# argsim/argsim

Measured on AMD Instinct MI355X. Metric: sentences/sec per ELBO step, higher is better.
Workload: dtype f32; 1 GPU; BASELINE configs[1]: 1xMI355X fp32, latent_dim 128, vocab 8k, seq_len 64, batch 256 per GPU; FULL synthetic Zipf batches, dim_emb 512, 3 layers, step 20000; global_batch=256, seq_len=64, parallelism=dp1, gru=persistent

## Files before the change

### argsim_amd/csrc/ctx.h

```cpp
#pragma once
#include "../../include/argsim_vae.h"
#include "kernels.h"

#include <fcntl.h>
#include <sys/file.h>
#include <unistd.h>

#include <algorithm>
#include <cmath>
#include <cstdio>
#include <cstring>
#include <string>
#include <vector>

#pragma GCC visibility push(hidden)
namespace avae { namespace host {

struct ParamEntry {
    std::string name;
    int64_t offset;
    int ndim;
    int64_t shape[4];
    int g16;
    int bucket;
// ... 7 lines not shown
struct avae_ctx {
    avae_config cfg{};
    int device = 0;
    hipStream_t stream = nullptr;
    std::string err;
    std::vector<avae::host::ParamEntry> params;
    int64_t numel = 0;
    std::vector<std::pair<int64_t, int64_t>> buckets;
    float *P = nullptr, *G = nullptr, *M = nullptr, *Vv = nullptr;
    int64_t step = 0;
    avae_grad_hook hook = nullptr; void* hook_user = nullptr;
    std::vector<int> hook_pending;
    int persistent = 1;
    bool first_step_checked = false;
    int gru_ablate = 0, gru_force_slow = 0, gru_stagger = 0, gru_item = 2;
    int skinny = 1;
    int score_plan[4] = {0, 0, 0, 0};
    const int* expect_ptr[3] = {nullptr, nullptr, nullptr}; int expect_val[3] = {0, 0, 0};
    int compact = 2;
    int skip_pad = 1;
    int shared_device = 0; int lock_fd = -1;
    int dyn_split = 1;
    int dyn_thin = 1;
    int enc_top1 = 1;
    int table_l1 = 1;
    int bf16_act = 1;
    int bf16_sv = 1;
    int bf16_tn = 1;
    int logits16 = 1;
    int bf16_nt8 = 1;
    int bf16_direct = 0;
    int gru_spec = 2;
    int bwd_rs = 2;
    int knn_chunk = 0;
    int gru_bf16 = 1;
    int64_t oE = 0, oKout = 0, oBout = 0, oWmu = 0, oBmu = 0, oWlv = 0, oBlv = 0, oWex = 0, oBex = 0;
    std::vector<avae::host::GruP> enc;
    std::vector<avae::host::GruP> dec;
    float* losses = nullptr;
    float* acc = nullptr;
    int* errw = nullptr;
    unsigned* counters = nullptr;
    float* scratch = nullptr;
    int64_t scratch_n = 0;
    char* ws = nullptr; size_t ws_cap = 0;
    int B = 0, Ss = 0, St = 0;
    int timing = 0, timing_on = 0;
    unsigned short *bfA = nullptr, *bfB = nullptr; size_t bfA_cap = 0, bfB_cap = 0;
    float* slab = nullptr; size_t slab_floats = 0;
    unsigned short* bfP = nullptr; size_t bfP_cap = 0;
    struct Stamp { hipEvent_t a, b; int cls; double flops; const int* dyn; int dyn_max; };
    std::vector<Stamp> stamps; size_t stamps_used = 0;
    int32_t* hint_dev = nullptr; volatile int32_t* hint_host = nullptr;
    const int32_t *cnt_src = nullptr, *cnt_tgt = nullptr;
};

#pragma GCC visibility push(hidden)
namespace avae { namespace host {

#define AV_CHECK(expr)                                                                              \
    do { hipError_t e_ = (expr); if (e_ != hipSuccess) {                                            \
        char b_[512]; snprintf(b_, sizeof b_, "%s:%d: %s -> %s", __FILE__, __LINE__, #expr, hipGetErrorString(e_)); \
        h->err = b_; return 1; } } while (0)
#define AV_TRY(expr) do { int r_ = (expr); if (r_) return r_; } while (0)

inline int fail(avae_ctx* h, const std::string& m) { h->err = m; return 1; }

#define AV_GRU(expr)                                                                                                \
    do { hipError_t e_ = (expr);                                                                                    \
         if (e_ == hipErrorCooperativeLaunchTooLarge)                                                               \
             return fail(h, "persistent GRU kernel: its workgroups cannot all be resident on this device at once (occupancy query x CU count < grid); " \
                            "run with avae_set_option(\"persistent\", 0)");                                         \
         if (e_ != hipSuccess) { char b_[512]; snprintf(b_, sizeof b_, "%s:%d: %s -> %s", __FILE__, __LINE__, #expr, hipGetErrorString(e_)); \
             h->err = b_; return 1; } } while (0)

struct DeviceTurn {
    avae_ctx* h; bool held = false;
    explicit DeviceTurn(avae_ctx* h_) : h(h_) {
        if (!h->shared_device || !h->persistent) return;
        if (h->lock_fd < 0) {
            char path[64]; snprintf(path, sizeof path, "/tmp/argsim_vae_dev%d.lock", h->device);
            h->lock_fd = open(path, O_CREAT | O_RDWR, 0666);
        }
        if (h->lock_fd >= 0 && flock(h->lock_fd, LOCK_EX) == 0) held = true;
    }
    ~DeviceTurn() { if (held) { (void)hipStreamSynchronize(h->stream); (void)flock(h->lock_fd, LOCK_UN); } }
};

struct Timed {
    avae_ctx* h; avae_ctx::Stamp* s = nullptr;
    Timed(avae_ctx* h_, int cls, double flops, const int* dyn = nullptr, int dyn_max = 0) : h(h_) {
        if (!h->timing) return;
        if (h->stamps_used == h->stamps.size()) {
            avae_ctx::Stamp n{};
            if (hipEventCreate(&n.a) != hipSuccess || hipEventCreate(&n.b) != hipSuccess) return;
            h->stamps.push_back(n);
        }
        s = &h->stamps[h->stamps_used++];
        s->cls = cls; s->flops = flops; s->dyn = dyn; s->dyn_max = dyn_max;
        (void)hipEventRecord(s->a, h->stream);
    }
    ~Timed() { if (s) (void)hipEventRecord(s->b, h->stream); }
};

struct Ws {
    int32_t *src_tm, *lens_src, *lens_tgt, *lead, *gold, *rank, *cidx, *ntok, *pred;
    float *emb_src, *emb_tgt, *ew, *dew;
    std::vector<float*> e_gi, e_hs, e_sv[2], e_hp[2];
    std::vector<float*> d_gi, d_hd, d_sv, d_hp;
    float *hpick, *mu, *lv, *z, *eps, *kld, *h0;
    float *xlast, *gib, *svb, *dgib, *dghb, *dxl;
    float *hc, *ho, *logits;
    float *loss_samp, *errt_samp;
    float *dho, *dhc, *dhd[2], *dgi_d, *dgh_d, *dh0, *carry, *dh0sum, *dz, *dmu, *dlv, *dhpick;
    float *dhs[2], *dgi_e, *dgh_e, *demb_src, *demb_tgt;
    std::vector<unsigned short*> e_hs16, d_hd16, e_hp16[2], d_hp16;
    std::vector<char> act_e, act_d, acth_e, acth_d;
    std::vector<unsigned short*> x16_e, x16_d;
    const unsigned short* x16_kept_e(int i) const { return x16_valid ? x16_e[i] : nullptr; }
    const unsigned short* x16_kept_d(int i) const { return x16_valid ? x16_d[i] : nullptr; }
    bool x16_valid = false;
    unsigned short *dgi16_d, *dgh16_d, *dgi16_e, *dgh16_e;
// ... 108 lines not shown
```

### argsim_amd/csrc/gemm_f32.hip

```cpp
#include "kernels.h"
#include <cstdlib>
#include <type_traits>

namespace avae {

typedef float f32x16 __attribute__((ext_vector_type(16)));

constexpr int BK = 32;
constexpr int LDK = BK + 4;

template <bool XC, int ROWS>
__device__ __forceinline__ void load_tile(float4 (&r)[ROWS / 32], const float* __restrict__ P, int ld,
                                          int x0, int X, int k0, int K1, int tid)
{
#pragma unroll
    for (int rep = 0; rep < ROWS / 32; ++rep) {
        int f = tid + 256 * rep;
        float4 v = make_float4(0.f, 0.f, 0.f, 0.f);
        if (XC) {
            int k = k0 + f / (ROWS / 4), x = x0 + ((f % (ROWS / 4)) << 2);
            if (k < K1 && x < X) v = *reinterpret_cast<const float4*>(P + (size_t)k * ld + x);
        } else {
            int x = x0 + (f >> 3), k = k0 + ((f & 7) << 2);
            if (x < X && k < K1) v = *reinterpret_cast<const float4*>(P + (size_t)x * ld + k);
// ... 77 lines not shown
        return;
    }
#pragma unroll
    for (int j = 0; j < TN; ++j) {
        int col = n0 + 32 * (wn * TN + j) + l31;
        if (col >= g.N) continue;
        float bv = add_bias ? g.bias[col] : 0.f;
#pragma unroll
        for (int i = 0; i < TM; ++i) {
#pragma unroll
            for (int r = 0; r < 16; ++r) {
                int row = m0 + 32 * (wm * TM + i) + (r & 3) + 8 * (r >> 2) + 4 * h;
                if (row >= M) continue;
                float v = g.alpha * acc[i][j][r] + bv;
                float* c = g.C + (size_t)row * g.ldc + col;
                if (atomic) atomicAdd(c, v);
                else if (g.accumulate) *c += v;
                else *c = v;
            }
        }
    }
}

template <bool A_MC, bool B_NC, int WM, int WN, int TM, int TN, bool FAST = false, bool DB = false>
__global__ __launch_bounds__(256, DB ? 2 : 3) void gemm_f32_kernel(GemmArgs g)
{
    constexpr int BM = 32 * WM * TM, BN = 32 * WN * TN;
    constexpr int kStage = (BM + BN) * LDK;
    __shared__ __attribute__((aligned(16))) float smem[kStage * (DB ? 2 : 1)];
    float* As = smem;
    float* Bs = smem + BM * LDK;

    const int tid = threadIdx.x, lane = tid & 63, wave = tid >> 6;
    const int h = lane >> 5, l31 = lane & 31;
    const int wm = wave / WN, wn = wave % WN;

    if (blockIdx.y) { g.A = g.A2; g.B = g.B2; g.C = g.C2; g.bias = g.bias2; }
    int M = g.M, K = g.K;
    if (g.dyn_kind == 1) M = min(M, *g.dyn);
    if (g.dyn_kind == 2) K = min(K, *g.dyn);

    const int tiles_n = (g.N + BN - 1) / BN;
    const int nblk = ((M + BM - 1) / BM) * tiles_n;
    int bid = blockIdx.x;
    {
        int q = nblk >> 3, r = nblk & 7, xcd = bid & 7, slot = bid >> 3;
        if (slot >= q + (xcd < r ? 1 : 0)) return;
        bid = (xcd < r ? xcd * (q + 1) : r * (q + 1) + (xcd - r) * q) + slot;
    }
    const int tm = bid / tiles_n, tn = bid - tm * tiles_n;
    const int m0 = tm * BM, n0 = tn * BN;
    if (m0 >= M) return;

    int kb = 0, ke = K;
    if (g.split_k > 1) {
        int ktiles = (K + BK - 1) / BK;
        int per = (ktiles + g.split_k - 1) / g.split_k;
        kb = blockIdx.z * per * BK;
        ke = min(K, kb + per * BK);
        if (kb >= ke) return;
// ... 88 lines not shown
}

template <bool A_MC, bool B_NC, bool FAST>
__global__ __launch_bounds__(256, 3) void gemm_f32_persist_kernel(GemmArgs g)
{
    static_assert(FAST, "buffer-load staging only (register budget of three workgroups per CU)");
    constexpr int TM = 2, TN = 2, WN = 2, BM = 128, BN = 128;
    __shared__ __attribute__((aligned(16))) float smem[(BM + BN) * LDK];
    float* As = smem;
    float* Bs = smem + BM * LDK;
    const int tid = threadIdx.x, lane = tid & 63, wave = tid >> 6;
    const int h = lane >> 5, l31 = lane & 31;
    const int wm = wave / WN, wn = wave % WN;

    int M = g.M;
    const int K = g.K;
    if (g.dyn_kind == 1) M = min(M, *g.dyn);
    const int tiles_n = (g.N + BN - 1) / BN;
    const int nblk = ((M + BM - 1) / BM) * tiles_n;
    const int xcd = blockIdx.x & 7, per_xcd = gridDim.x >> 3;
    const int q = nblk >> 3, r = nblk & 7;
    const int run0 = xcd < r ? xcd * (q + 1) : r * (q + 1) + (xcd - r) * q, run_n = q + (xcd < r ? 1 : 0);
    int local = blockIdx.x >> 3;
    if (local >= run_n) return;

    float4 ra[BM / 32], rb[BN / 32];
    FastTile<A_MC, BM> fa; FastTile<B_NC, BN> fb;
    auto first_tile = [&](int bid) __attribute__((always_inline)) {
        const int tm = bid / tiles_n, tn = bid - tm * tiles_n;
        if (FAST) {
            fa.init(g.A, g.lda, tm * BM, M, 0, K, tid); fb.init(g.B, g.ldb, tn * BN, g.N, 0, K, tid);
            fa.load(ra, 0); fb.load(rb, 0);
        } else {
            load_tile<A_MC, BM>(ra, g.A, g.lda, tm * BM, M, 0, K, tid);
            load_tile<B_NC, BN>(rb, g.B, g.ldb, tn * BN, g.N, 0, K, tid);
        }
    };
    first_tile(run0 + local);
    for (; local < run_n; local += per_xcd) {
        const int bid = run0 + local;
        const int tm = bid / tiles_n, tn = bid - tm * tiles_n;
        const int m0 = tm * BM, n0 = tn * BN;
        const bool more = local + per_xcd < run_n;
        f32x16 acc[TM][TN];
#pragma unroll
        for (int i = 0; i < TM; ++i)
#pragma unroll
            for (int j = 0; j < TN; ++j)
#pragma unroll
                for (int e = 0; e < 16; ++e) acc[i][j][e] = 0.f;
        for (int k0 = 0; k0 < K; k0 += BK) {
            store_tile<A_MC, BM>(As, ra, tid);
            store_tile<B_NC, BN>(Bs, rb, tid);
            if (k0 + BK < K) {
                if (FAST) { const int it = k0 / BK + 1; fa.load(ra, it); fb.load(rb, it); }
                else {
                    load_tile<A_MC, BM>(ra, g.A, g.lda, m0, M, k0 + BK, K, tid);
                    load_tile<B_NC, BN>(rb, g.B, g.ldb, n0, g.N, k0 + BK, K, tid);
                }
            } else if (more) {
                first_tile(bid + per_xcd);
// ... 16 lines not shown
#pragma unroll
                for (int t = 0; t < TN; ++t) {
                    if (B_NC) {
#pragma unroll
                        for (int e = 0; e < 4; ++e) b[t][e] = Bs[(8 * qq + 4 * h + e) * BN + 32 * (wn * TN + t) + l31];
                    } else {
                        float4 v = *reinterpret_cast<const float4*>(Bs + (32 * (wn * TN + t) + l31) * LDK + 8 * qq + 4 * h);
                        b[t][0] = v.x; b[t][1] = v.y; b[t][2] = v.z; b[t][3] = v.w;
                    }
                }
#pragma unroll
                for (int e = 0; e < 4; ++e)
#pragma unroll
                    for (int i = 0; i < TM; ++i)
#pragma unroll
                        for (int j = 0; j < TN; ++j)
                            acc[i][j] = __builtin_amdgcn_mfma_f32_32x32x2f32(a[i][e], b[j][e], acc[i][j], 0, 0, 0);
            }
            __builtin_amdgcn_s_setprio(0);
            __syncthreads();
        }
        epilogue<TM, TN, WN>(g, acc, M, m0, n0, BM, BN, wm, wn, h, l31, false, g.bias != nullptr);
    }
}

template <bool B_NC>
__global__ __launch_bounds__(512) void gemm_f32_skinny_kernel(GemmArgs g)
{
    __shared__ float red[7][16][64];
    if (blockIdx.y) { g.A = g.A2; g.B = g.B2; g.C = g.C2; g.bias = g.bias2; }
    const int tid = threadIdx.x, lane = tid & 63, wave = tid >> 6, l31 = lane & 31, h = lane >> 5;
    const int tiles_n = (g.N + 31) / 32, tm = blockIdx.x / tiles_n, tn = blockIdx.x - tm * tiles_n;
    const int m0 = tm * 32, n0 = tn * 32;
    const int kchunk = ((g.K + 63) / 64) * 8;
    const int k0 = wave * kchunk, k1 = min(g.K, k0 + kchunk);
    const float* __restrict__ ap = g.A + (size_t)min(m0 + l31, g.M - 1) * g.lda;
    const int bcol = min(n0 + l31, g.N - 1);
    const float* __restrict__ bp = B_NC ? g.B + bcol : g.B + (size_t)bcol * g.ldb;
    f32x16 acc;
#pragma unroll
    for (int r = 0; r < 16; ++r) acc[r] = 0.f;
    for (int kk = k0; kk < k1; kk += 32) {
        float4 a[4], b[4];
#pragma unroll
        for (int u = 0; u < 4; ++u) {
            const int k = kk + 8 * u + 4 * h;
// ... 40 lines not shown
    return !a_mc && g.split_k <= 1 && g.dyn_kind == 0 && (g.K & 3) == 0 && (g.lda & 3) == 0 && g.K >= 64;
}
static void launch_skinny(hipStream_t st, bool b_nc, const GemmArgs& g)
{
    dim3 grid(((g.M + 31) / 32) * ((g.N + 31) / 32), g.A2 ? 2 : 1);
    if (b_nc) hipLaunchKernelGGL(gemm_f32_skinny_kernel<true>, grid, dim3(512), 0, st, g);
    else      hipLaunchKernelGGL(gemm_f32_skinny_kernel<false>, grid, dim3(512), 0, st, g);
}

template <class F>
static void with_layouts(bool a_mc, bool b_nc, F&& f)
{
    if (!a_mc && !b_nc)      f(std::false_type{}, std::false_type{});
    else if (!a_mc && b_nc)  f(std::false_type{}, std::true_type{});
    else if (a_mc && b_nc)   f(std::true_type{}, std::true_type{});
    else                     f(std::true_type{}, std::false_type{});
}

template <int WM, int WN, int TM, int TN>
static void launch_variant(hipStream_t st, bool a_mc, bool b_nc, const GemmArgs& g)
{
    constexpr int BM = 32 * WM * TM, BN = 32 * WN * TN;
    int tiles = ((g.M + BM - 1) / BM) * ((g.N + BN - 1) / BN);
    dim3 grid(tiles, g.A2 ? 2 : 1, g.split_k > 1 ? g.split_k : 1);
    static const bool allow_fast = !getenv("AVAE_F32_NOFAST");
    const int k_per_wg = g.split_k > 1 ? (g.K + g.split_k - 1) / g.split_k : g.K;
    const bool fast = allow_fast && (a_mc ? (g.M % BM == 0) : (g.K % BK == 0 && g.dyn_kind != 2)) &&
                      (b_nc ? (g.N % BN == 0) : (g.K % BK == 0 && g.dyn_kind != 2)) && (a_mc || b_nc || k_per_wg >= 1536);
    static const char* ps_env = getenv("AVAE_F32_PERSIST");
    if constexpr (WM == 2 && WN == 2) {
        const bool aligned = (a_mc ? (g.M % BM == 0) : (g.K % BK == 0)) && (b_nc ? (g.N % BN == 0) : (g.K % BK == 0));
        const bool persist = (ps_env ? atoi(ps_env) != 0 : true) && allow_fast && aligned && !g.A2 && g.split_k <= 1 && g.dyn_kind != 2 && tiles > 1024;
        if (persist) {
            dim3 pg(768);
            with_layouts(a_mc, b_nc, [&](auto A, auto B) { hipLaunchKernelGGL((gemm_f32_persist_kernel<decltype(A)::value, decltype(B)::value, true>), pg, dim3(256), 0, st, g); });
            return;
        }
    }
    static const char* db_env = getenv("AVAE_F32_DB");
    if constexpr (WM == 2 && WN == 2) {
        const int eff_tiles = (g.dyn_kind == 1 && g.dyn_expect > 0) ? std::min(tiles, ((g.dyn_expect + BM - 1) / BM) * ((g.N + BN - 1) / BN)) : (g.dyn_kind == 1 ? 0 : tiles);
        const bool use_db = db_env ? atoi(db_env) != 0 && !g.A2 : (!g.A2 && g.split_k <= 1 && eff_tiles > 768 && tiles <= 1024);
        if (use_db) {
            if (fast) {
                with_layouts(a_mc, b_nc, [&](auto A, auto B) { hipLaunchKernelGGL((gemm_f32_kernel<decltype(A)::value, decltype(B)::value, WM, WN, TM, TN, true, true>), grid, dim3(256), 0, st, g); });
            } else {
                with_layouts(a_mc, b_nc, [&](auto A, auto B) { hipLaunchKernelGGL((gemm_f32_kernel<decltype(A)::value, decltype(B)::value, WM, WN, TM, TN, false, true>), grid, dim3(256), 0, st, g); });
            }
            return;
        }
    }
    if (fast) {
        with_layouts(a_mc, b_nc, [&](auto A, auto B) { hipLaunchKernelGGL((gemm_f32_kernel<decltype(A)::value, decltype(B)::value, WM, WN, TM, TN, true>), grid, dim3(256), 0, st, g); });
        return;
    }
    with_layouts(a_mc, b_nc, [&](auto A, auto B) { hipLaunchKernelGGL((gemm_f32_kernel<decltype(A)::value, decltype(B)::value, WM, WN, TM, TN>), grid, dim3(256), 0, st, g); });
}

hipError_t gemm_f32(hipStream_t st, bool a_mc, bool b_nc, const GemmArgs& g)
{
    if (g.M <= 0 || g.N <= 0) return hipSuccess;
    if ((g.lda | g.ldb) & 3) return hipErrorInvalidValue;
    if (((uintptr_t)g.A | (uintptr_t)g.B | (uintptr_t)g.A2 | (uintptr_t)g.B2) & 15) return hipErrorInvalidValue;
    if (!a_mc && (g.K & 3)) return hipErrorInvalidValue;
    if (a_mc && (g.M & 3)) return hipErrorInvalidValue;
    if (!b_nc && (g.K & 3)) return hipErrorInvalidValue;
    if (b_nc && (g.N & 3)) return hipErrorInvalidValue;
    if (g.thin == 3 && skinny_ok(a_mc, g) && (b_nc || (g.ldb & 3) == 0)) launch_skinny(st, b_nc, g);
    else if (g.thin == 3) launch_variant<1, 4, 1, 1>(st, a_mc, b_nc, g);
    else if (g.thin == 2) launch_variant<2, 2, 1, 1>(st, a_mc, b_nc, g);
    else if (g.thin) launch_variant<1, 4, 1, 1>(st, a_mc, b_nc, g);
    else        launch_variant<2, 2, 2, 2>(st, a_mc, b_nc, g);
    return hipGetLastError();
}

}
```

### argsim_amd/csrc/gemm_plan.cpp

```cpp
#include "gemm_plan.h"

#include <algorithm>
#include <cmath>

namespace avae {

namespace {

GemmPlan one(const GemmShape& s, int thin, int split_k, int accumulate, int zero = kZeroNone, bool dyn = true)
{
    return GemmPlan{1, {{0, s.M, thin, split_k, accumulate, zero, dyn && s.dyn_kind ? 1 : 0}, {0, 0, 0, 0, 0, 0, 0}}};
}

int grad_split(int M, int N, int K)
{
    int tiles = ((M + 127) / 128) * ((N + 127) / 128);
    int s = 768 / tiles;
    int kmax = K / 128; if (kmax < 1) kmax = 1;
    if (s > kmax) s = kmax;
    return s < 1 ? 1 : s;
}

GemmPlan plan_wgrad(const GemmShape& s)
{
// ... 42 lines not shown
        const int sk = std::min(4, K / 768);
        if (s.allow_atomic && s.dyn_split && plain_out && sk >= 2) return one(s, 2, sk, 0, kZeroDynRows);
        return one(s, 2, 1, s.accumulate);
    }
    if (s.dyn_thin && s.dyn_kind == 1 && s.compute_dtype == 0 && tiles <= 768 && nt > 4 && K <= 512 && !s.accumulate) return one(s, 1, 1, s.accumulate);
    if (tiles > 256 && tiles % 256 != 0) {
        int main_mt = mt;
        while (main_mt > 0 && (main_mt * nt) % 256 != 0) --main_mt;
        const int tail_tiles = (mt - main_mt) * nt;
        const double frac = (double)tiles / 256.0;
        if (main_mt > 0 && tail_tiles < 200 && (std::ceil(frac) - frac) >= 0.3) {
            const int main_rows = main_mt * 128, tail_rows = M - main_rows;
            GemmPlan p{2, {{0, main_rows, 0, 1, s.accumulate, kZeroNone, s.dyn_kind ? 1 : 0}, {main_rows, tail_rows, thin_form, 1, s.accumulate, kZeroNone, 0}}};
            if (s.allow_atomic && plain_out && K >= 1024 && !(s.skinny && K <= 2048 && s.compute_dtype != 1)) {
                const int sk = std::min(768 / (((tail_rows + 127) / 128) * nt), K / 128);
                if (sk >= 2) p.launch[1] = GemmLaunch{main_rows, tail_rows, 0, sk, 0, kZeroAll, 0};
            }
            return p;
        }
    }
    return one(s, 0, 1, s.accumulate);
}

bool gemm_tn16_shape(int M, int N) { return ((M | N) & 7) == 0 && (long long)M * N >= 1ll << 19; }

int gemm_bf16_slices(int split_k, int big_tiles, int K, int bk)
{
    const int s2 = split_k > 1 ? (512 + big_tiles / 2) / big_tiles : 1;
    return std::max(1, std::min(std::min(s2, 16), std::max(1, K / (4 * bk))));
}
bool gemm_bf16_big_fills(int M, int N, int big_tiles, int slices) { return N >= 192 && M >= 192 && big_tiles * slices >= 200; }

}
```

### argsim_amd/csrc/gemm_plan.h

```cpp
#pragma once

namespace avae {

struct GemmShape {
    bool a_mc, b_nc;
    int M, N, K, ldc;
    int accumulate;
    int split_k;
    int thin;
    int dyn_kind, dyn_expect;
    bool allow_atomic;
    bool rows_are_batch;
    bool pair;
    bool wgrad;
    int compute_dtype;
    bool skinny, dyn_split, dyn_thin;
};
enum GemmZero { kZeroNone = 0, kZeroAll = 1, kZeroDynRows = 2 };
struct GemmLaunch {
    int row0, rows;
    int thin, split_k, accumulate;
    int zero;
    int dyn;
};
struct GemmPlan { int n; GemmLaunch launch[2]; };
GemmPlan gemm_plan(const GemmShape& s);

bool gemm_tn16_shape(int M, int N);
int gemm_bf16_slices(int split_k, int big_tiles, int K, int bk);
bool gemm_bf16_big_fills(int M, int N, int big_tiles, int slices);

}
```

### argsim_amd/csrc/handle.cpp

```cpp
#include "ctx.h"

using namespace avae;
using namespace avae::host;

static std::string g_create_err;

namespace avae { namespace host {

int grow_scratch(avae_ctx* h, size_t need, const char* what)
{
    if (h->scratch_n >= (int64_t)need) return 0;
    AV_CHECK(hipStreamSynchronize(h->stream));
    if (h->scratch) AV_CHECK(hipFree(h->scratch));
    h->scratch = nullptr; h->scratch_n = 0;
    if (hipMalloc(reinterpret_cast<void**>(&h->scratch), need) != hipSuccess) {
        (void)hipGetLastError();
        h->scratch = nullptr;
        char b_[256]; snprintf(b_, sizeof b_, "%s: %.0f MB of scratch could not be allocated on the device", what, (double)need / 1048576.0);
        return fail(h, b_);
    }
    h->scratch_n = (int64_t)need;
    return 0;
}

// ... 207 lines not shown
int avae_set_grad_hook(avae_handle h, avae_grad_hook hook, void* user) { if (!h) return 1; h->hook = hook; h->hook_user = user; return 0; }

int avae_set_option(avae_handle h, const char* key, int value)
{
    if (!h || !key) return 1;
    if (!strcmp(key, "persistent")) { h->persistent = value; return 0; }
    if (!strcmp(key, "gru_item")) { h->gru_item = value; return 0; }
    if (!strcmp(key, "gru_stagger")) { h->gru_stagger = value; return 0; }
    if (!strcmp(key, "gru_force_slow")) { h->gru_force_slow = value; return 0; }
    if (!strcmp(key, "gru_bf16")) { h->gru_bf16 = value != 0; return 0; }
    if (!strcmp(key, "bwd_rs")) { h->bwd_rs = value; return 0; }
    if (!strcmp(key, "dyn_split")) { h->dyn_split = value != 0; return 0; }
    if (!strcmp(key, "shared_device")) { h->shared_device = value != 0; return 0; }
    if (!strcmp(key, "gru_spec")) { h->gru_spec = value; return 0; }
    if (!strcmp(key, "bf16_nt8")) { h->bf16_nt8 = value != 0; return 0; }
    if (!strcmp(key, "logits16")) { h->logits16 = value != 0; return 0; }
    if (!strcmp(key, "bf16_direct")) { h->bf16_direct = value != 0; return 0; }
    if (!strcmp(key, "bf16_tn")) { h->bf16_tn = value != 0; return 0; }
    if (!strcmp(key, "bf16_sv")) { h->bf16_sv = value != 0; return 0; }
    if (!strcmp(key, "bf16_act")) { h->bf16_act = value != 0; return 0; }
    if (!strcmp(key, "table_l1")) { h->table_l1 = value != 0; return 0; }
    if (!strcmp(key, "enc_top1")) { h->enc_top1 = value != 0; return 0; }
    if (!strcmp(key, "dyn_thin")) { h->dyn_thin = value != 0; return 0; }
    if (!strcmp(key, "skip_pad")) { h->skip_pad = value != 0; return 0; }
    if (!strcmp(key, "compact")) { h->compact = value; return 0; }
    if (!strcmp(key, "skinny")) { h->skinny = value; return 0; }
    if (!strcmp(key, "knn_chunk")) { if (value < 0) return fail(h, "knn_chunk must be >= 0"); h->knn_chunk = value; return 0; }
    if (!strcmp(key, "gru_ablate")) {
        if (value && !gru_diag_build()) return fail(h, "gru_ablate needs the diagnostic build of libargsim_vae.so (make -C argsim_amd/csrc DIAG=1)");
        h->gru_ablate = value; return 0;
    }
    if (!strcmp(key, "timing")) { h->timing = value; h->timing_on = value; h->stamps_used = 0; return 0; }
    if (!strcmp(key, "timing_pause")) { h->timing = value ? 0 : h->timing_on; return 0; }
    return fail(h, "unknown option");
}
int avae_timing_collect(avae_handle h, double* out)
{
    if (!h || !out) return 1;
    AV_CHECK(hipStreamSynchronize(h->stream));
    for (int i = 0; i < 9; ++i) out[i] = 0.0;
    std::vector<std::pair<const int*, int>> seen;
    for (size_t i = 0; i < h->stamps_used; ++i) {
        float ms = 0.f;
        AV_CHECK(hipEventElapsedTime(&ms, h->stamps[i].a, h->stamps[i].b));
        double f = 1.0;
        AV_TRY(dyn_fraction(h, h->stamps[i], seen, &f));
        int c = h->stamps[i].cls;
        out[3 * c] += ms; out[3 * c + 1] += 1.0; out[3 * c + 2] += h->stamps[i].flops * f;
    }
    h->stamps_used = 0;
    return 0;
}
int avae_bucket_count(avae_handle h) { return h ? (int)h->buckets.size() : 0; }
int avae_bucket_info(avae_handle h, int i, int64_t* offset, int64_t* count)
{
    if (!h || i < 0 || i >= (int)h->buckets.size()) return 1;
    *offset = h->buckets[i].first; *count = h->buckets[i].second; return 0;
}

}
```

### argsim_amd/csrc/hooks.cpp

```cpp
#include "ctx.h"

using namespace avae;
using namespace avae::host;

extern "C" {

int avae_debug_team_batch(int32_t B) { return B > 0 ? gru_team_batch(B) : 0; }
int avae_debug_gemm_plan(const int32_t* in, int32_t n, int32_t* out)
{
    if (!in || !out || n < 0) return 1;
    for (int r = 0; r < n; ++r, in += 19, out += 15) {
        const GemmShape s{in[0] != 0, in[1] != 0, in[2], in[3], in[4], in[5], in[6], in[7], in[8], in[9], in[10], in[11] != 0, in[12] != 0,
                          in[13] != 0, in[14] != 0, in[15], in[16] != 0, in[17] != 0, in[18] != 0};
        const GemmPlan p = gemm_plan(s);
        out[0] = p.n;
        for (int i = 0; i < 2; ++i) {
            const GemmLaunch l = i < p.n ? p.launch[i] : GemmLaunch{0, 0, 0, 0, 0, 0, 0};
            const int32_t f[7] = {l.row0, l.rows, l.thin, l.split_k, l.accumulate, l.zero, l.dyn};
            std::copy(f, f + 7, out + 1 + 7 * i);
        }
    }
    return 0;
}
int avae_debug_gemm_call(avae_handle h, int a_mc, int b_nc, const float* A, const float* Bm, float* Cm, const float* bias, int M, int N, int K,
                         int lda, int ldb, int ldc, float alpha, int accumulate, int flags, const int* count, int expect,
                         const float* A2, const float* B2, float* C2, unsigned short* keep16)
{
    if (!h) return 1;
    GemmCall c{A, lda, a_mc != 0, Bm, ldb, b_nc != 0, Cm, ldc, M, N, K};
    c.alpha = alpha; c.bias = bias; c.accumulate = accumulate; c.keep_a16 = keep16;
    c.allow_atomic = (flags & 1) != 0; c.rows_are_batch = (flags & 2) != 0; c.wgrad = (flags & 4) != 0;
    if (c.wgrad) c.depth(count); else c.rows(count);
    const Pair second{A2, B2, C2, nullptr};
    if (A2) c.pair = &second;
    const int* const was_ptr = h->expect_ptr[0]; const int was_val = h->expect_val[0];
    h->expect_ptr[0] = count; h->expect_val[0] = expect;
    const int r = gemm(h, c);
    h->expect_ptr[0] = was_ptr; h->expect_val[0] = was_val;
    return r;
}
int avae_debug_score_plan(avae_handle h, int32_t out[4])
{
    if (!h || !out) return 1;
    for (int i = 0; i < 4; ++i) out[i] = h->score_plan[i];
    return 0;
}
// ... 11 lines not shown
    if (!h || !out || !n_out) return 1;
    if (h->B < 1) return fail(h, "avae_debug_train_ce: no training forward has run on this handle");
    Ws w;
    AV_TRY(get_ws(h, w, h->B, h->Ss, h->St, true));
    int n = 0;
    AV_CHECK(hipMemcpyAsync(&n, w.ntok, sizeof(int), hipMemcpyDeviceToHost, h->stream));
    AV_CHECK(hipStreamSynchronize(h->stream));
    n = std::min(n, (int)max_n);
    AV_CHECK(hipMemcpyAsync(out, w.loss_samp, (size_t)n * sizeof(float), hipMemcpyDeviceToDevice, h->stream));
    *n_out = n;
    return 0;
}
int avae_debug_timing(avae_handle h, double* out, int max_n, int* n)
{
    if (!h || !out || !n) return 1;
    AV_CHECK(hipStreamSynchronize(h->stream));
    *n = (int)std::min<size_t>(h->stamps_used, (size_t)max_n);
    std::vector<std::pair<const int*, int>> seen;
    for (int i = 0; i < *n; ++i) {
        float ms = 0.f;
        AV_CHECK(hipEventElapsedTime(&ms, h->stamps[i].a, h->stamps[i].b));
        double f = 1.0;
        AV_TRY(dyn_fraction(h, h->stamps[i], seen, &f));
        const double fl = h->stamps[i].flops * f;
        out[3 * i] = h->stamps[i].cls; out[3 * i + 1] = ms; out[3 * i + 2] = fl;
    }
    return 0;
}
int avae_debug_stamps(avae_handle h, unsigned long long* out)
{
    if (!h || !out) return 1;
    AV_CHECK(hipStreamSynchronize(h->stream));
    AV_CHECK(hipMemcpy(out, h->errw + 16, 32 * sizeof(unsigned long long), hipMemcpyDeviceToHost));
    AV_CHECK(hipMemset(h->errw + 16, 0, 32 * sizeof(unsigned long long)));
    return 0;
}
int avae_debug_gemm(avae_handle h, int a_mc, int b_nc, const float* A, const float* Bm, float* Cm, const float* bias,
                    int M, int N, int K, int lda, int ldb, int ldc, float alpha, int accumulate, int split_k)
{
    if (!h) return 1;
    GemmCall c{A, lda, a_mc != 0, Bm, ldb, b_nc != 0, Cm, ldc, M, N, K};
    c.alpha = alpha; c.bias = bias; c.accumulate = accumulate;
    return gemm(h, c.form(split_k == -3 ? 3 : (split_k < 0 ? 1 : (split_k >= 1000 ? 2 : 0)), split_k < 0 ? 1 : (split_k >= 1000 ? split_k - 1000 : split_k)));
}
int avae_debug_gemm_dyn(avae_handle h, const float* A, const float* Bm, float* Cm, int M, int N, int K, const int* rows)
{
    if (!h) return 1;
// ... 147 lines not shown
```

### argsim_amd/csrc/kernels.h

```cpp
#pragma once
#include <hip/hip_runtime.h>
#include <stdint.h>

#include "gemm_plan.h"

namespace avae {

struct GemmArgs {
    const float* A; const float* B; float* C; const float* bias;
    int M, N, K, lda, ldb, ldc;
    float alpha;
    int accumulate;
    int split_k;
    const int* dyn; int dyn_kind;
    int dyn_expect;
    int thin;
    const float* A2; const float* B2; float* C2; const float* bias2;
    float* slab = nullptr; size_t slab_floats = 0;
    unsigned short* c16 = nullptr;
    int nt8 = 1;
};
hipError_t gemm_f32(hipStream_t st, bool a_mc, bool b_nc, const GemmArgs& g);
hipError_t gemm_f32s(hipStream_t st, bool a_mc, bool b_nc, const GemmArgs& g);
hipError_t gemm_bf16_direct(hipStream_t st, bool a_mc, bool b_nc, const GemmArgs& g);

hipError_t cvt_bf16(hipStream_t st, const float* src, int ld, bool transpose, int rows_or_K, int cols_or_X,
                    unsigned short* dst, int ldd);
hipError_t gemm_bf16_nt(hipStream_t st, const unsigned short* A, int lda, const unsigned short* B, int ldb, const GemmArgs& g);
bool gemm_bf16_p8_ok(const GemmArgs& g, int lda, int ldb);
hipError_t gemm_bf16_p8(hipStream_t st, const unsigned short* A, int lda, const unsigned short* B, int ldb, const GemmArgs& g, int s2);
bool gemm_bf16_c16_ok(const GemmArgs& g, int lda, int ldb);
bool gemm_bf16_c16_takes(int M, int N, int K, const int* rows, int nt8);
bool gemm_bf16_p8_tn_ok(const GemmArgs& g, int lda, int ldb);
hipError_t gemm_bf16_p8_tn(hipStream_t st, const unsigned short* A, int lda, const unsigned short* B, int ldb, const GemmArgs& g, int s2);
hipError_t gemm_bf16_tn(hipStream_t st, const unsigned short* A, int lda, const unsigned short* B, int ldb, const GemmArgs& g);
hipError_t transpose_bf16(hipStream_t st, const unsigned short* src, int ld, int K, int X, unsigned short* dst, int ldk);

constexpr int kMaxGruJobs = 3;
struct GruJob {
    const float* gi;
    const int32_t* gi_rows;
    const float* R;
    const float* bR;
// ... 228 lines not shown
```

### argsim_amd/csrc/model.cpp

```cpp
#include "ctx.h"

using namespace avae;

namespace avae { namespace host {

static bool phantom_batch(const avae_ctx* h, int B)
{
    return h->compact && h->skip_pad && h->persistent && h->cfg.dim_emb == 512 && gru_team_batch(B) > B;
}
bool use_table(const avae_ctx* h, int rows, int B)
{
    if (!h->table_l1 || !id_groups_supported(h->cfg.dim_tgt)) return false;
    return rows >= h->cfg.dim_tgt || (rows >= 1024 && phantom_batch(h, B));
}

void layout(avae_ctx* h, Bump& b, Ws& w, int B, int Ss, int St, bool train)
{
    const int D = h->cfg.dim_emb, V = h->cfg.dim_tgt, R = h->cfg.dim_rep, L = h->cfg.rnn_layers;
    const size_t T = St + 1, rs = (size_t)Ss * B, rt = T * B;
    w.src_tm = b.take<int32_t>(rs); w.lens_src = b.take<int32_t>(B); w.lens_tgt = b.take<int32_t>(B);
    w.lead = b.take<int32_t>(rt); w.gold = b.take<int32_t>(rt); w.rank = b.take<int32_t>(rt);
    w.cidx = b.take<int32_t>(rt); w.ntok = b.take<int32_t>(4 + kPrepChunks); w.pred = b.take<int32_t>(rt);
    w.emb_src = b.take<float>(rs * D); w.emb_tgt = b.take<float>(rt * D);
    const bool tab_s = use_table(h, (int)rs, B), tab_t = use_table(h, (int)rt, B);
// ... 104 lines not shown
    return 0;
}

static int dyn_expected(const avae_ctx* h, const int* dyn, int dyn_kind)
{
    if (dyn_kind != 1 || !dyn) return 0;
    for (int i = 0; i < 3; ++i) if (dyn == h->expect_ptr[i]) return h->expect_val[i];
    return 0;
}

static GemmShape gemm_shape(const avae_ctx* h, const GemmCall& c)
{
    return GemmShape{c.a_mc, c.b_nc, c.M, c.N, c.K, c.ldc, c.accumulate, c.split_k, c.thin, c.dyn_kind, dyn_expected(h, c.dyn, c.dyn_kind),
                     c.allow_atomic, c.rows_are_batch, c.pair != nullptr, c.wgrad, h->cfg.compute_dtype, h->skinny != 0, h->dyn_split != 0, h->dyn_thin != 0};
}
static GemmLaunch bf16_launch(const avae_ctx* h, const GemmCall& c)
{
    if (!c.wgrad) return GemmLaunch{0, c.M, 0, 1, c.accumulate, kZeroNone, c.dyn_kind ? 1 : 0};
    GemmShape s = gemm_shape(h, c);
    s.compute_dtype = 1;
    return gemm_plan(s).launch[0];
}

static int gemm_launch(avae_ctx* h, const GemmCall& c, const GemmLaunch& l)
{
    if (c.pair && h->cfg.compute_dtype != 0) {
        GemmCall one = c, two = c;
        one.pair = two.pair = nullptr; two.keep_a16 = nullptr;
        two.A = c.pair->A; two.B = c.pair->B; two.C = c.pair->C; two.bias = c.pair->bias;
        AV_TRY(gemm_launch(h, one, l));
        return gemm_launch(h, two, l);
    }
    const float* A = c.A + (size_t)l.row0 * c.lda; float* C = c.C + (size_t)l.row0 * c.ldc;
    const int M = l.rows, N = c.N, K = c.K;
    const int* dyn = l.dyn ? c.dyn : nullptr; const int dyn_kind = l.dyn ? c.dyn_kind : 0;
    const Pair* pair = c.pair;
    GemmArgs g{A, c.B, C, c.bias, M, N, K, c.lda, c.ldb, c.ldc, c.alpha, l.accumulate, l.split_k, dyn, dyn_kind, dyn_expected(h, dyn, dyn_kind), l.thin,
               pair ? pair->A : nullptr, pair ? pair->B : nullptr, pair ? pair->C : nullptr, pair ? pair->bias : nullptr};
    Timed t(h, 0, 2.0 * M * N * K * (pair ? 2 : 1), dyn, dyn_kind == 1 ? M : (dyn_kind == 2 ? K : 0));
    if (h->cfg.compute_dtype == 1 && h->bf16_direct) {
        AV_CHECK(gemm_bf16_direct(h->stream, c.a_mc, c.b_nc, g));
        return 0;
    }
    if (h->cfg.compute_dtype == 1) {
        const int Kp = (K + 7) & ~7;
        unsigned short* a16 = nullptr;
        if (c.keep_a16 && !c.a_mc && Kp == K) a16 = c.keep_a16 + (size_t)l.row0 * K;
        if (!a16) { AV_TRY(grow_bf16(h, &h->bfA, &h->bfA_cap, (size_t)M * Kp)); a16 = h->bfA; }
        AV_TRY(grow_bf16(h, &h->bfB, &h->bfB_cap, (size_t)N * Kp));
        AV_CHECK(cvt_bf16(h->stream, A, c.lda, c.a_mc, c.a_mc ? K : M, c.a_mc ? M : K, a16, Kp));
        AV_CHECK(cvt_bf16(h->stream, c.B, c.ldb, c.b_nc, c.b_nc ? K : N, c.b_nc ? N : K, h->bfB, Kp));
        g.nt8 = h->bf16_nt8;
        g.c16 = c.c16;
        AV_CHECK(gemm_bf16_nt(h->stream, a16, Kp, h->bfB, Kp, g));
        return 0;
    }
    if (c.c16) return fail(h, "the fp16 output panel exists in compute_dtype 1 only");
    if (h->cfg.compute_dtype == 2 && !l.thin) AV_CHECK(gemm_f32s(h->stream, c.a_mc, c.b_nc, g));
    else AV_CHECK(gemm_f32(h->stream, c.a_mc, c.b_nc, g));
    return 0;
}

int gemm(avae_ctx* h, const GemmCall& c)
{
    const GemmPlan p = gemm_plan(gemm_shape(h, c));
    for (int i = 0; i < p.n; ++i) {
        const GemmLaunch& l = p.launch[i];
        float* C = c.C + (size_t)l.row0 * c.ldc;
        if (l.zero == kZeroAll) AV_CHECK(zero_fill(h->stream, C, sizeof(float) * (size_t)l.rows * c.N));
        if (l.zero == kZeroDynRows) AV_CHECK(zero_rows_dyn(h->stream, C, c.dyn, l.rows, c.N));
        AV_TRY(gemm_launch(h, c, l));
    }
    return 0;
}

static int gemm_bf16_pre(avae_ctx* h, const GemmCall& c)
{
    const GemmLaunch l = bf16_launch(h, c);
    const int M = c.M, N = c.N, K = c.K;
    GemmArgs g{nullptr, c.B, c.C, c.bias, M, N, K, c.lda, c.ldb, c.ldc, c.alpha, l.accumulate, l.split_k, c.dyn, c.dyn_kind, 0, 0, nullptr, nullptr, nullptr, nullptr};
    Timed t(h, 0, 2.0 * M * N * K, c.dyn, c.dyn_kind == 1 ? M : (c.dyn_kind == 2 ? K : 0));
    const int Kp = (K + 7) & ~7;
    const unsigned short* Ap = c.A16; int lda_p = c.lda;
    if (c.a_mc) {
        AV_TRY(grow_bf16(h, &h->bfA, &h->bfA_cap, (size_t)M * Kp));
        AV_CHECK(transpose_bf16(h->stream, c.A16, c.lda, K, M, h->bfA, Kp));
        Ap = h->bfA; lda_p = Kp;
    }
// ... 700 lines not shown
```

### argsim_amd/lib.py

```python
import ctypes as C
import os
import subprocess

_HERE = os.path.dirname(os.path.abspath(__file__))
LIB_PATH = os.path.join(_HERE, 'libargsim_vae.so')
CSRC = os.path.join(_HERE, 'csrc')


def source_digest():
    import glob
    import hashlib
    h = hashlib.sha1()
    files = sorted(glob.glob(os.path.join(CSRC, '*.hip')) + glob.glob(os.path.join(CSRC, '*.cpp')) + glob.glob(os.path.join(CSRC, '*.h')))
    files.append(os.path.join(os.path.dirname(_HERE), 'include', 'argsim_vae.h'))
    for f in files:
        h.update(os.path.basename(f).encode())
        with open(f, 'rb') as fh:
            h.update(fh.read())
    return h.hexdigest()[:16]


class AvaeConfig(C.Structure):
    _fields_ = [('dim_tgt', C.c_int32), ('dim_emb', C.c_int32), ('dim_rep', C.c_int32), ('rnn_layers', C.c_int32),
                ('accelerate', C.c_float), ('learn_rate', C.c_float), ('bos', C.c_int32), ('eos', C.c_int32),
# ... 57 lines not shown
    'avae_score': (C.c_int, [_P, _P, _P, C.c_int32, C.c_int32, C.c_int32, C.POINTER(AvaeScoreConfig), _P, _P, _P, _P, _P, _P]),
    'avae_score_z': (C.c_int, [_P, _P, _P, C.c_int32, C.c_int32, _P, _P]),
    'avae_knn': (C.c_int, [_P, _P, C.c_int32, _P, C.c_int32, C.c_int32, C.POINTER(AvaeKnnConfig), _P, _P]),
    'avae_set_option': (C.c_int, [_P, C.c_char_p, C.c_int]),
    'avae_debug_gemm': (C.c_int, [_P, C.c_int, C.c_int, _P, _P, _P, _P] + [C.c_int] * 6 + [C.c_float, C.c_int, C.c_int]),
    'avae_debug_gemm_dyn': (C.c_int, [_P, _P, _P, _P, C.c_int, C.c_int, C.c_int, _P]),
    'avae_debug_gemm_c16': (C.c_int, [_P, _P, _P, _P, C.c_int, C.c_int, C.c_int, C.c_float, _P]),
    'avae_debug_gemm_tn16': (C.c_int, [_P, _P, _P, _P] + [C.c_int] * 6 + [C.c_float]),
    'avae_debug_softmax_ce': (C.c_int, [_P, _P, _P, C.c_int, _P, _P, _P, C.c_int, C.c_int, C.c_int, C.c_float, _P, _P, _P, C.POINTER(C.c_int)]),
    'avae_debug_argmax_rows': (C.c_int, [_P, _P, _P, C.c_int, C.c_int]),
    'avae_debug_op': (C.c_int, [_P, C.c_char_p, C.POINTER(_P), C.POINTER(C.c_int64), C.POINTER(C.c_float)]),
    'avae_debug_op_layout': (C.c_int, [C.c_int64, C.c_int64, C.POINTER(C.c_int64)]),
    'avae_debug_sample_rows': (C.c_int, [_P, _P, C.c_int, C.c_int, C.c_int, C.POINTER(AvaeSampleConfig), _P, _P]),
    'avae_debug_sample_rows_p': (C.c_int, [_P, _P, C.c_int, C.c_int, C.c_int, C.POINTER(AvaeSamplePConfig), _P, _P, _P, _P]),
    'avae_debug_beam_select': (C.c_int, [_P, _P, C.c_int, C.c_int, C.c_int, _P, _P, _P, _P, _P, _P]),
    'avae_timing_collect': (C.c_int, [_P, C.POINTER(C.c_double)]),
    'avae_debug_timing': (C.c_int, [_P, C.POINTER(C.c_double), C.c_int, C.POINTER(C.c_int)]),
    'avae_debug_train_ce': (C.c_int, [_P, _P, C.c_int32, C.POINTER(C.c_int32)]),
    'avae_debug_stamps': (C.c_int, [_P, C.POINTER(C.c_uint64)]),
    'avae_debug_present_ids': (C.c_int, [_P, C.POINTER(C.c_int32)]),
    'avae_debug_score_plan': (C.c_int, [_P, C.POINTER(C.c_int32)]),
    'avae_debug_team_batch': (C.c_int, [C.c_int32]),
    'avae_debug_gemm_plan': (C.c_int, [_P, C.c_int32, _P]),
    'avae_debug_gemm_call': (C.c_int, [_P, C.c_int, C.c_int, _P, _P, _P, _P] + [C.c_int] * 6 + [C.c_float, C.c_int, C.c_int, _P, C.c_int, _P, _P, _P, _P]),
    'avae_bucket_count': (C.c_int, [_P]),
    'avae_bucket_info': (C.c_int, [_P, C.c_int, C.POINTER(C.c_int64), C.POINTER(C.c_int64)]),
}

_lib = None


def build(force=False, jobs=4):
    if force:
        subprocess.run(['make', '-C', CSRC, 'clean'], check=True, stdout=subprocess.DEVNULL)
    subprocess.run(['make', '-C', CSRC, '-j%d' % jobs], check=True, stdout=subprocess.DEVNULL)
    return LIB_PATH


def load():
    global _lib
    if _lib is not None:
        return _lib
    if not os.path.exists(LIB_PATH):
        raise RuntimeError("libargsim_vae.so is not built: run `python -c 'import __graft_entry__ as g; g.build()'` "
                           "(there is no CPU fallback for the HIP path)")
    lib = C.CDLL(LIB_PATH)
# ... 7 lines not shown
```

Before: 15410 sentences/sec.

## Fuse GEMM row-tail launch into the main 128x128 tile kernel

When a GEMM plan splits into a main 128-row-aligned launch and a thin tail launch, the tail rows are now computed inside the same kernel. Extra workgroups, or the leftover iterations of the persistent loop, run a 32x128 tail tile. This removes a second kernel launch and the serialization between the two launches, and the tail work can overlap with the main tiles. In exchange it adds code paths to the main kernel, which can raise register pressure, and the timing stamps gain a fixed-flops field.

After: 15430 sentences/sec, median of 2. Within noise of the previous version (+0.1%).

```diff
diff --git a/argsim_amd/csrc/ctx.h b/argsim_amd/csrc/ctx.h
--- a/argsim_amd/csrc/ctx.h
+++ b/argsim_amd/csrc/ctx.h
@@ -53,6 +53,7 @@
     int shared_device = 0; int lock_fd = -1;
     int dyn_split = 1;
     int dyn_thin = 1;
+    int fuse_tail = 1;
     int enc_top1 = 1;
     int table_l1 = 1;
     int bf16_act = 1;
@@ -80,7 +81,7 @@
     unsigned short *bfA = nullptr, *bfB = nullptr; size_t bfA_cap = 0, bfB_cap = 0;
     float* slab = nullptr; size_t slab_floats = 0;
     unsigned short* bfP = nullptr; size_t bfP_cap = 0;
-    struct Stamp { hipEvent_t a, b; int cls; double flops; const int* dyn; int dyn_max; };
+    struct Stamp { hipEvent_t a, b; int cls; double flops; const int* dyn; int dyn_max; double flops_fixed; };
     std::vector<Stamp> stamps; size_t stamps_used = 0;
     int32_t* hint_dev = nullptr; volatile int32_t* hint_host = nullptr;
     const int32_t *cnt_src = nullptr, *cnt_tgt = nullptr;
@@ -120,7 +121,7 @@
 
 struct Timed {
     avae_ctx* h; avae_ctx::Stamp* s = nullptr;
-    Timed(avae_ctx* h_, int cls, double flops, const int* dyn = nullptr, int dyn_max = 0) : h(h_) {
+    Timed(avae_ctx* h_, int cls, double flops, const int* dyn = nullptr, int dyn_max = 0, double flops_fixed = 0.0) : h(h_) {
         if (!h->timing) return;
         if (h->stamps_used == h->stamps.size()) {
             avae_ctx::Stamp n{};
@@ -128,7 +129,7 @@
             h->stamps.push_back(n);
         }
         s = &h->stamps[h->stamps_used++];
-        s->cls = cls; s->flops = flops; s->dyn = dyn; s->dyn_max = dyn_max;
+        s->cls = cls; s->flops = flops; s->dyn = dyn; s->dyn_max = dyn_max; s->flops_fixed = flops_fixed;
         (void)hipEventRecord(s->a, h->stream);
     }
     ~Timed() { if (s) (void)hipEventRecord(s->b, h->stream); }
diff --git a/argsim_amd/csrc/gemm_f32.hip b/argsim_amd/csrc/gemm_f32.hip
--- a/argsim_amd/csrc/gemm_f32.hip
+++ b/argsim_amd/csrc/gemm_f32.hip
@@ -123,6 +123,66 @@
     }
 }
 
+template <bool A_MC, bool B_NC, bool FAST>
+__device__ __forceinline__ void tail_tile(const GemmArgs& g, float* smem, int t, int tid)
+{
+    constexpr int BM = 32, BN = 128;
+    float* As = smem;
+    float* Bs = smem + BM * LDK;
+    const int lane = tid & 63, wn = tid >> 6, h = lane >> 5, l31 = lane & 31;
+    const int tiles_n = (g.N + BN - 1) / BN;
+    const int tm = t / tiles_n, tn = t - tm * tiles_n;
+    const int m0 = g.tail_row0 + tm * BM, n0 = tn * BN, M = g.tail_row0 + g.tail_rows, K = g.K;
+    f32x16 acc[1][1];
+#pragma unroll
+    for (int r = 0; r < 16; ++r) acc[0][0][r] = 0.f;
+    float4 ra[BM / 32], rb[BN / 32];
+    FastTile<A_MC, BM> fa; FastTile<B_NC, BN> fb;
+    if (FAST) {
+        fa.init(g.A, g.lda, m0, M, 0, K, tid); fb.init(g.B, g.ldb, n0, g.N, 0, K, tid);
+        fa.load(ra, 0); fb.load(rb, 0);
+    } else {
+        load_tile<A_MC, BM>(ra, g.A, g.lda, m0, M, 0, K, tid);
+        load_tile<B_NC, BN>(rb, g.B, g.ldb, n0, g.N, 0, K, tid);
+    }
+    for (int k0 = 0; k0 < K; k0 += BK) {
+        store_tile<A_MC, BM>(As, ra, tid);
+        store_tile<B_NC, BN>(Bs, rb, tid);
+        if (k0 + BK < K) {
+            if (FAST) { const int it = k0 / BK + 1; fa.load(ra, it); fb.load(rb, it); }
+            else {
+                load_tile<A_MC, BM>(ra, g.A, g.lda, m0, M, k0 + BK, K, tid);
+                load_tile<B_NC, BN>(rb, g.B, g.ldb, n0, g.N, k0 + BK, K, tid);
+            }
+        }
+        __syncthreads();
+        __builtin_amdgcn_s_setprio(1);
+#pragma unroll
+        for (int q = 0; q < 4; ++q) {
+            float a[4], b[4];
+            if (A_MC) {
+#pragma unroll
+                for (int e = 0; e < 4; ++e) a[e] = As[(8 * q + 4 * h + e) * BM + l31];
+            } else {
+                const float4 v = *reinterpret_cast<const float4*>(As + l31 * LDK + 8 * q + 4 * h);
+                a[0] = v.x; a[1] = v.y; a[2] = v.z; a[3] = v.w;
+            }
+            if (B_NC) {
+#pragma unroll
+                for (int e = 0; e < 4; ++e) b[e] = Bs[(8 * q + 4 * h + e) * BN + 32 * wn + l31];
+            } else {
+                const float4 v = *reinterpret_cast<const float4*>(Bs + (32 * wn + l31) * LDK + 8 * q + 4 * h);
+                b[0] = v.x; b[1] = v.y; b[2] = v.z; b[3] = v.w;
+            }
+#pragma unroll
+            for (int e = 0; e < 4; ++e) acc[0][0] = __builtin_amdgcn_mfma_f32_32x32x2f32(a[e], b[e], acc[0][0], 0, 0, 0);
+        }
+        __builtin_amdgcn_s_setprio(0);
+        __syncthreads();
+    }
+    epilogue<1, 1, 4>(g, acc, M, m0, n0, BM, BN, 0, wn, h, l31, false, g.bias != nullptr);
+}
+
 template <bool A_MC, bool B_NC, int WM, int WN, int TM, int TN, bool FAST = false, bool DB = false>
 __global__ __launch_bounds__(256, DB ? 2 : 3) void gemm_f32_kernel(GemmArgs g)
 {
@@ -137,6 +197,13 @@
     const int wm = wave / WN, wn = wave % WN;
 
     if (blockIdx.y) { g.A = g.A2; g.B = g.B2; g.C = g.C2; g.bias = g.bias2; }
+    if constexpr (BM == 128 && BN == 128 && !A_MC) {
+        const int main_grid = ((g.M + BM - 1) / BM) * ((g.N + BN - 1) / BN);
+        if (g.tail_rows > 0 && (int)blockIdx.x >= main_grid) {
+            tail_tile<A_MC, B_NC, FAST>(g, smem, blockIdx.x - main_grid, tid);
+            return;
+        }
+    }
     int M = g.M, K = g.K;
     if (g.dyn_kind == 1) M = min(M, *g.dyn);
     if (g.dyn_kind == 2) K = min(K, *g.dyn);
@@ -271,7 +338,7 @@
     const int q = nblk >> 3, r = nblk & 7;
     const int run0 = xcd < r ? xcd * (q + 1) : r * (q + 1) + (xcd - r) * q, run_n = q + (xcd < r ? 1 : 0);
     int local = blockIdx.x >> 3;
-    if (local >= run_n) return;
+    if (local >= run_n && (A_MC || g.tail_rows <= 0)) return;
 
     float4 ra[BM / 32], rb[BN / 32];
     FastTile<A_MC, BM> fa; FastTile<B_NC, BN> fb;
@@ -285,7 +352,7 @@
             load_tile<B_NC, BN>(rb, g.B, g.ldb, tn * BN, g.N, 0, K, tid);
         }
     };
-    first_tile(run0 + local);
+    if (local < run_n) first_tile(run0 + local);
     for (; local < run_n; local += per_xcd) {
         const int bid = run0 + local;
         const int tm = bid / tiles_n, tn = bid - tm * tiles_n;
@@ -348,6 +415,16 @@
         }
         epilogue<TM, TN, WN>(g, acc, M, m0, n0, BM, BN, wm, wn, h, l31, false, g.bias != nullptr);
     }
+    if constexpr (!A_MC) {
+        if (g.tail_rows > 0) {
+            const int ttiles = ((g.tail_rows + g.tail_bm - 1) / g.tail_bm) * tiles_n;
+            const int tq = ttiles >> 3, tr = ttiles & 7;
+            const int trun0 = xcd < tr ? xcd * (tq + 1) : tr * (tq + 1) + (xcd - tr) * tq, trun_n = tq + (xcd < tr ? 1 : 0);
+            int ttid = tid;
+            asm volatile("" : "+v"(ttid));
+            for (int tl = local - run_n; tl < trun_n; tl += per_xcd) tail_tile<A_MC, B_NC, FAST>(g, smem, trun0 + tl, ttid);
+        }
+    }
 }
 
 template <bool B_NC>
@@ -434,7 +511,8 @@
 {
     constexpr int BM = 32 * WM * TM, BN = 32 * WN * TN;
     int tiles = ((g.M + BM - 1) / BM) * ((g.N + BN - 1) / BN);
-    dim3 grid(tiles, g.A2 ? 2 : 1, g.split_k > 1 ? g.split_k : 1);
+    const int tail_tiles = g.tail_rows > 0 ? ((g.tail_rows + g.tail_bm - 1) / g.tail_bm) * ((g.N + BN - 1) / BN) : 0;
+    dim3 grid(tiles + tail_tiles, g.A2 ? 2 : 1, g.split_k > 1 ? g.split_k : 1);
     static const bool allow_fast = !getenv("AVAE_F32_NOFAST");
     const int k_per_wg = g.split_k > 1 ? (g.K + g.split_k - 1) / g.split_k : g.K;
     const bool fast = allow_fast && (a_mc ? (g.M % BM == 0) : (g.K % BK == 0 && g.dyn_kind != 2)) &&
@@ -478,6 +556,7 @@
     if (a_mc && (g.M & 3)) return hipErrorInvalidValue;
     if (!b_nc && (g.K & 3)) return hipErrorInvalidValue;
     if (b_nc && (g.N & 3)) return hipErrorInvalidValue;
+    if (g.tail_rows > 0 && (g.thin || a_mc || g.split_k > 1 || g.A2 || g.dyn_kind == 2 || g.tail_bm != 32 || g.tail_row0 < g.M)) return hipErrorInvalidValue;
     if (g.thin == 3 && skinny_ok(a_mc, g) && (b_nc || (g.ldb & 3) == 0)) launch_skinny(st, b_nc, g);
     else if (g.thin == 3) launch_variant<1, 4, 1, 1>(st, a_mc, b_nc, g);
     else if (g.thin == 2) launch_variant<2, 2, 1, 1>(st, a_mc, b_nc, g);
diff --git a/argsim_amd/csrc/gemm_plan.cpp b/argsim_amd/csrc/gemm_plan.cpp
--- a/argsim_amd/csrc/gemm_plan.cpp
+++ b/argsim_amd/csrc/gemm_plan.cpp
@@ -88,6 +88,16 @@
     return one(s, 0, 1, s.accumulate);
 }
 
+bool gemm_tail_fusable(const GemmShape& s, const GemmPlan& p)
+{
+    if (p.n != 2 || s.compute_dtype != 0 || s.a_mc || s.pair || s.wgrad || s.dyn_kind == 2) return false;
+    const GemmLaunch& m = p.launch[0];
+    const GemmLaunch& t = p.launch[1];
+    if (m.row0 != 0 || m.rows <= 0 || m.rows % 128 != 0 || m.thin != 0 || m.split_k != 1 || m.zero != kZeroNone) return false;
+    if (t.row0 != m.rows || t.rows <= 0 || t.row0 + t.rows != s.M) return false;
+    return t.thin == 1 && t.split_k == 1 && t.zero == kZeroNone && t.dyn == 0 && t.accumulate == m.accumulate;
+}
+
 bool gemm_tn16_shape(int M, int N) { return ((M | N) & 7) == 0 && (long long)M * N >= 1ll << 19; }
 
 int gemm_bf16_slices(int split_k, int big_tiles, int K, int bk)
diff --git a/argsim_amd/csrc/gemm_plan.h b/argsim_amd/csrc/gemm_plan.h
--- a/argsim_amd/csrc/gemm_plan.h
+++ b/argsim_amd/csrc/gemm_plan.h
@@ -25,6 +25,7 @@
 };
 struct GemmPlan { int n; GemmLaunch launch[2]; };
 GemmPlan gemm_plan(const GemmShape& s);
+bool gemm_tail_fusable(const GemmShape& s, const GemmPlan& p);
 
 bool gemm_tn16_shape(int M, int N);
 int gemm_bf16_slices(int split_k, int big_tiles, int K, int bk);
diff --git a/argsim_amd/csrc/handle.cpp b/argsim_amd/csrc/handle.cpp
--- a/argsim_amd/csrc/handle.cpp
+++ b/argsim_amd/csrc/handle.cpp
@@ -253,6 +253,7 @@
     if (!strcmp(key, "table_l1")) { h->table_l1 = value != 0; return 0; }
     if (!strcmp(key, "enc_top1")) { h->enc_top1 = value != 0; return 0; }
     if (!strcmp(key, "dyn_thin")) { h->dyn_thin = value != 0; return 0; }
+    if (!strcmp(key, "fuse_tail")) { h->fuse_tail = value != 0; return 0; }
     if (!strcmp(key, "skip_pad")) { h->skip_pad = value != 0; return 0; }
     if (!strcmp(key, "compact")) { h->compact = value; return 0; }
     if (!strcmp(key, "skinny")) { h->skinny = value; return 0; }
@@ -277,7 +278,7 @@
         double f = 1.0;
         AV_TRY(dyn_fraction(h, h->stamps[i], seen, &f));
         int c = h->stamps[i].cls;
-        out[3 * c] += ms; out[3 * c + 1] += 1.0; out[3 * c + 2] += h->stamps[i].flops * f;
+        out[3 * c] += ms; out[3 * c + 1] += 1.0; out[3 * c + 2] += h->stamps[i].flops * f + h->stamps[i].flops_fixed;
     }
     h->stamps_used = 0;
     return 0;
diff --git a/argsim_amd/csrc/hooks.cpp b/argsim_amd/csrc/hooks.cpp
--- a/argsim_amd/csrc/hooks.cpp
+++ b/argsim_amd/csrc/hooks.cpp
@@ -22,6 +22,16 @@
     }
     return 0;
 }
+int avae_debug_gemm_fusable(const int32_t* in, int32_t n, int32_t* out)
+{
+    if (!in || !out || n < 0) return 1;
+    for (int r = 0; r < n; ++r, in += 19) {
+        const GemmShape s{in[0] != 0, in[1] != 0, in[2], in[3], in[4], in[5], in[6], in[7], in[8], in[9], in[10], in[11] != 0, in[12] != 0,
+                          in[13] != 0, in[14] != 0, in[15], in[16] != 0, in[17] != 0, in[18] != 0};
+        out[r] = gemm_tail_fusable(s, gemm_plan(s)) ? 1 : 0;
+    }
+    return 0;
+}
 int avae_debug_gemm_call(avae_handle h, int a_mc, int b_nc, const float* A, const float* Bm, float* Cm, const float* bias, int M, int N, int K,
                          int lda, int ldb, int ldc, float alpha, int accumulate, int flags, const int* count, int expect,
                          const float* A2, const float* B2, float* C2, unsigned short* keep16)
@@ -79,7 +89,7 @@
         AV_CHECK(hipEventElapsedTime(&ms, h->stamps[i].a, h->stamps[i].b));
         double f = 1.0;
         AV_TRY(dyn_fraction(h, h->stamps[i], seen, &f));
-        const double fl = h->stamps[i].flops * f;
+        const double fl = h->stamps[i].flops * f + h->stamps[i].flops_fixed;
         out[3 * i] = h->stamps[i].cls; out[3 * i + 1] = ms; out[3 * i + 2] = fl;
     }
     return 0;
diff --git a/argsim_amd/csrc/kernels.h b/argsim_amd/csrc/kernels.h
--- a/argsim_amd/csrc/kernels.h
+++ b/argsim_amd/csrc/kernels.h
@@ -19,6 +19,7 @@
     float* slab = nullptr; size_t slab_floats = 0;
     unsigned short* c16 = nullptr;
     int nt8 = 1;
+    int tail_row0 = 0, tail_rows = 0, tail_bm = 32;
 };
 hipError_t gemm_f32(hipStream_t st, bool a_mc, bool b_nc, const GemmArgs& g);
 hipError_t gemm_f32s(hipStream_t st, bool a_mc, bool b_nc, const GemmArgs& g);
diff --git a/argsim_amd/csrc/model.cpp b/argsim_amd/csrc/model.cpp
--- a/argsim_amd/csrc/model.cpp
+++ b/argsim_amd/csrc/model.cpp
@@ -150,7 +150,7 @@
     return gemm_plan(s).launch[0];
 }
 
-static int gemm_launch(avae_ctx* h, const GemmCall& c, const GemmLaunch& l)
+static int gemm_launch(avae_ctx* h, const GemmCall& c, const GemmLaunch& l, const GemmLaunch* tail = nullptr)
 {
     if (c.pair && h->cfg.compute_dtype != 0) {
         GemmCall one = c, two = c;
@@ -165,7 +165,8 @@
     const Pair* pair = c.pair;
     GemmArgs g{A, c.B, C, c.bias, M, N, K, c.lda, c.ldb, c.ldc, c.alpha, l.accumulate, l.split_k, dyn, dyn_kind, dyn_expected(h, dyn, dyn_kind), l.thin,
                pair ? pair->A : nullptr, pair ? pair->B : nullptr, pair ? pair->C : nullptr, pair ? pair->bias : nullptr};
-    Timed t(h, 0, 2.0 * M * N * K * (pair ? 2 : 1), dyn, dyn_kind == 1 ? M : (dyn_kind == 2 ? K : 0));
+    if (tail) { g.tail_row0 = tail->row0 - l.row0; g.tail_rows = tail->rows; g.tail_bm = 32; }
+    Timed t(h, 0, 2.0 * M * N * K * (pair ? 2 : 1), dyn, dyn_kind == 1 ? M : (dyn_kind == 2 ? K : 0), tail ? 2.0 * tail->rows * N * K : 0.0);
     if (h->cfg.compute_dtype == 1 && h->bf16_direct) {
         AV_CHECK(gemm_bf16_direct(h->stream, c.a_mc, c.b_nc, g));
         return 0;
@@ -191,7 +192,9 @@
 
 int gemm(avae_ctx* h, const GemmCall& c)
 {
-    const GemmPlan p = gemm_plan(gemm_shape(h, c));
+    const GemmShape s = gemm_shape(h, c);
+    const GemmPlan p = gemm_plan(s);
+    if (h->fuse_tail && gemm_tail_fusable(s, p)) return gemm_launch(h, c, p.launch[0], &p.launch[1]);
     for (int i = 0; i < p.n; ++i) {
         const GemmLaunch& l = p.launch[i];
         float* C = c.C + (size_t)l.row0 * c.ldc;
diff --git a/argsim_amd/lib.py b/argsim_amd/lib.py
--- a/argsim_amd/lib.py
+++ b/argsim_amd/lib.py
@@ -103,6 +103,7 @@
     'avae_debug_score_plan': (C.c_int, [_P, C.POINTER(C.c_int32)]),
     'avae_debug_team_batch': (C.c_int, [C.c_int32]),
     'avae_debug_gemm_plan': (C.c_int, [_P, C.c_int32, _P]),
+    'avae_debug_gemm_fusable': (C.c_int, [_P, C.c_int32, _P]),
     'avae_debug_gemm_call': (C.c_int, [_P, C.c_int, C.c_int, _P, _P, _P, _P] + [C.c_int] * 6 + [C.c_float, C.c_int, C.c_int, _P, C.c_int, _P, _P, _P, _P]),
     'avae_bucket_count': (C.c_int, [_P]),
     'avae_bucket_info': (C.c_int, [_P, C.c_int, C.POINTER(C.c_int64), C.POINTER(C.c_int64)]),
```
